# Mehooz/vision4leg

Measured on AMD Instinct MI355X. Metric: PPO env-steps/s (encoder+update, sim excluded), higher is better.
Workload: dtype f16; 1 GPU; ppo_locotransformer thin-goal: LocoTransformer S=93 A=6, E=32 envs x T=512, B=1024, 3 opt epochs; net=loco, envs_per_gpu=32, horizon=512, minibatch=1024, opt_epochs=3, parallelism=dp1, includes_rollout_inference=True, logp_old=recorded at action time (target_pf forward skipped; SURVEY 8d declared saving)

## Files before the change

vision4leg_amd/csrc/bwd.h:

```cpp
#pragma once
#include "infer.h"

namespace v4l {

struct BwdLayer {
  const void *w2t, *w1t, *wot, *wint;
  const float *g1, *g2;
  const float* dy;
  const float *s_qkv, *s_P, *s_xh1, *s_rs1, *s_xh2, *s_rs2;
  const void* s_f;
  void *o_dz2, *o_df, *o_dz1, *o_dqkv;
  float* o_dx;
  float *gp2, *bp2, *gp1, *bp1;
};

struct BwdLayerStack { BwdLayer l[2]; };

struct BwdHead {
  const void *w2t, *w1t, *w0t;
  const float* dout;
  const float *s_h1, *s_h0;
  float *o_dh1, *o_dh0;
};
struct BwdTail {
// ... 416 lines not shown
      f32x4 ap[2][2];
#pragma unroll
      for (int m = 0; m < 2; ++m)
#pragma unroll
        for (int nn = 0; nn < 2; ++nn) ap[m][nn] = f32x4{0.f, 0.f, 0.f, 0.f};
#pragma unroll
      for (int ks = 0; ks < 2; ++ks) {
        frag_t fa[2], fb[2];
#pragma unroll
        for (int m = 0; m < 2; ++m) {
          fa[m] = *reinterpret_cast<const frag_t*>(dC + (m * 16 + fr) * LY::LDA + ks * 32 + fg);
          fb[m] = *reinterpret_cast<const frag_t*>(Vv + (m * 16 + fr) * LY::LDA + ks * 32 + fg);
        }
#pragma unroll
        for (int m = 0; m < 2; ++m)
#pragma unroll
          for (int nn = 0; nn < 2; ++nn) mma_k32(ap[m][nn], fb[nn], fa[m]);
      }
#pragma unroll
      for (int m = 0; m < 2; ++m) {
        const int i = m * 16 + fr;
        float rd = 0.f;
#pragma unroll
        for (int nn = 0; nn < 2; ++nn)
#pragma unroll
          for (int r = 0; r < 4; ++r) {
            const bool ok = i < NTOK && nn * 16 + qr + r < NTOK;
            rd = fmaf(pp[m][nn][r], ok ? ap[m][nn][r] : 0.f, rd);
          }
        rd += __shfl_xor(rd, 16, 64);
        rd += __shfl_xor(rd, 32, 64);
#pragma unroll
        for (int nn = 0; nn < 2; ++nn) {
          float d[4];
#pragma unroll
          for (int r = 0; r < 4; ++r) {
            const bool ok = i < NTOK && nn * 16 + qr + r < NTOK;
            d[r] = ok ? pp[m][nn][r] * (ap[m][nn][r] - rd) : 0.f;
          }
          const int j0 = nn * 16 + qr;
          st4(dS + i * LY::LDK + j0, d[0], d[1], d[2], d[3]);
#pragma unroll
          for (int r = 0; r < 4; ++r) {
            dSt[(j0 + r) * LY::LDK + i] = (T)d[r];
            Pt[(j0 + r) * LY::LDK + i] = (T)pp[m][nn][r];
          }
        }
      }
      T* R = reinterpret_cast<T*>(aw);
      if (lane < LY::LDR * 2 / 16) *reinterpret_cast<uint4*>(R + NTOK * LY::LDR + lane * 8) = uint4{0u, 0u, 0u, 0u};
      T* og = reinterpret_cast<T*>(w.o_dqkv) + (row0 + wave * NTOK) * 192;
      auto product = [&](const T* A, const T* B, float scale, int coff) {
        f32x4 acc[2][4];
        frag_t fa[2], fb[4];
#pragma unroll
        for (int m = 0; m < 2; ++m) fa[m] = *reinterpret_cast<const frag_t*>(A + (m * 16 + fr) * LY::LDK + fg);
#pragma unroll
        for (int nn = 0; nn < 4; ++nn) fb[nn] = *reinterpret_cast<const frag_t*>(B + (nn * 16 + fr) * LY::LDK + fg);
#pragma unroll
        for (int m = 0; m < 2; ++m)
#pragma unroll
          for (int nn = 0; nn < 4; ++nn) {
            acc[m][nn] = f32x4{0.f, 0.f, 0.f, 0.f};
            mma_k32(acc[m][nn], fb[nn], fa[m]);
          }
#pragma unroll
        for (int m = 0; m < 2; ++m) {
          const int x = m * 16 + fr;
          if (x < NTOK) {
#pragma unroll
            for (int nn = 0; nn < 4; ++nn) {
              const float v0 = acc[m][nn][0] * scale, v1 = acc[m][nn][1] * scale, v2 = acc[m][nn][2] * scale, v3 = acc[m][nn][3] * scale;
              st4(R + x * LY::LDR + coff + nn * 16 + qr, v0, v1, v2, v3);
              st4(og + x * 192 + coff + nn * 16 + qr, v0, v1, v2, v3);
            }
          }
        }
      };
      product(dS, Kt, 0.125f, 0);
      product(dSt, Qt, 0.125f, TD);
      product(Pt, dCt, 1.f, 2 * TD);
    }
  } else {
    const bool act = wave < ns;
    float* qs = big + wave * NTOK * LY::LDQ;
    float* p = sp + wave * NTOK * ATT_PLD;
    float* ds = sp + (SPW + wave) * NTOK * ATT_PLD;
    const float* dc = a + wave * NTOK * LY::LDX;
    if (act) {
      if (lane < 54) {
        const int a2 = lane / 6, b3 = lane - a2 * 6;
        const int i0 = 2 * a2, i1 = min(i0 + 1, NTOK - 1), j0 = 3 * b3, j1 = min(j0 + 1, NTOK - 1), j2 = min(j0 + 2, NTOK - 1);
        const float *da = dc + i0 * LY::LDX, *db = dc + i1 * LY::LDX;
        const float *va = qs + j0 * LY::LDQ + 2 * TD, *vb = qs + j1 * LY::LDQ + 2 * TD, *vc = qs + j2 * LY::LDQ + 2 * TD;
        float s00 = 0.f, s01 = 0.f, s02 = 0.f, s10 = 0.f, s11 = 0.f, s12 = 0.f;
#pragma unroll 4
        for (int d = 0; d < TD; d += 4) {
          const float4 x0 = *reinterpret_cast<const float4*>(da + d), x1 = *reinterpret_cast<const float4*>(db + d);
          const float4 y0 = *reinterpret_cast<const float4*>(va + d), y1 = *reinterpret_cast<const float4*>(vb + d);
          const float4 y2 = *reinterpret_cast<const float4*>(vc + d);
          s00 = fmaf(x0.x, y0.x, s00); s00 = fmaf(x0.y, y0.y, s00); s00 = fmaf(x0.z, y0.z, s00); s00 = fmaf(x0.w, y0.w, s00);
          s01 = fmaf(x0.x, y1.x, s01); s01 = fmaf(x0.y, y1.y, s01); s01 = fmaf(x0.z, y1.z, s01); s01 = fmaf(x0.w, y1.w, s01);
          s02 = fmaf(x0.x, y2.x, s02); s02 = fmaf(x0.y, y2.y, s02); s02 = fmaf(x0.z, y2.z, s02); s02 = fmaf(x0.w, y2.w, s02);
          s10 = fmaf(x1.x, y0.x, s10); s10 = fmaf(x1.y, y0.y, s10); s10 = fmaf(x1.z, y0.z, s10); s10 = fmaf(x1.w, y0.w, s10);
          s11 = fmaf(x1.x, y1.x, s11); s11 = fmaf(x1.y, y1.y, s11); s11 = fmaf(x1.z, y1.z, s11); s11 = fmaf(x1.w, y1.w, s11);
          s12 = fmaf(x1.x, y2.x, s12); s12 = fmaf(x1.y, y2.y, s12); s12 = fmaf(x1.z, y2.z, s12); s12 = fmaf(x1.w, y2.w, s12);
        }
        float* r0 = ds + i0 * ATT_PLD;
        float* r1 = ds + i1 * ATT_PLD;
        r0[j0] = s00;
        if (j0 + 1 < NTOK) r0[j0 + 1] = s01;
        if (j0 + 2 < NTOK) r0[j0 + 2] = s02;
        if (i0 + 1 < NTOK) {
          r1[j0] = s10;
          if (j0 + 1 < NTOK) r1[j0 + 1] = s11;
          if (j0 + 2 < NTOK) r1[j0 + 2] = s12;
        }
      }
      if (lane < 3 * NTOK) {
        const int i = lane / 3, j = NTOK + lane - i * 3;
        p[i * ATT_PLD + j] = 0.f;
        ds[i * ATT_PLD + j] = 0.f;
      }
    }
    __syncthreads();
    if (act && lane < NTOK) {
      float rd = 0.f;
#pragma unroll
      for (int j = 0; j < NTOK; ++j) rd = fmaf(p[lane * ATT_PLD + j], ds[lane * ATT_PLD + j], rd);
#pragma unroll
      for (int j = 0; j < NTOK; ++j) {
        const float pj = p[lane * ATT_PLD + j];
        ds[lane * ATT_PLD + j] = rt<T>(pj * (ds[lane * ATT_PLD + j] - rd));
        p[lane * ATT_PLD + j] = rt<T>(pj);
      }
    }
    __syncthreads();
    if (act) {
      float dcr[NTOK], kr[NTOK], qq[NTOK], dq[NTOK], dk[NTOK], dv[NTOK];
#pragma unroll
      for (int i = 0; i < NTOK; ++i) {
        dcr[i] = dc[i * LY::LDX + lane];
        qq[i] = qs[i * LY::LDQ + lane];
        kr[i] = qs[i * LY::LDQ + TD + lane];
        dq[i] = dk[i] = dv[i] = 0.f;
      }
#pragma unroll
      for (int i = 0; i < NTOK; ++i) {
        float pi[ATT_PLD], si[ATT_PLD];
#pragma unroll
        for (int j4 = 0; j4 < ATT_PLD; j4 += 4) {
          const float4 pv = *reinterpret_cast<const float4*>(p + i * ATT_PLD + j4);
          const float4 sv = *reinterpret_cast<const float4*>(ds + i * ATT_PLD + j4);
          pi[j4] = pv.x; pi[j4 + 1] = pv.y; pi[j4 + 2] = pv.z; pi[j4 + 3] = pv.w;
          si[j4] = sv.x; si[j4 + 1] = sv.y; si[j4 + 2] = sv.z; si[j4 + 3] = sv.w;
        }
#pragma unroll
        for (int j = 0; j < NTOK; ++j) {
          dv[j] = fmaf(pi[j], dcr[i], dv[j]);
          dq[i] = fmaf(si[j], kr[j], dq[i]);
          dk[j] = fmaf(si[j], qq[i], dk[j]);
        }
      }
      T* og = reinterpret_cast<T*>(w.o_dqkv) + (row0 + wave * NTOK) * 192;
#pragma unroll
      for (int i = 0; i < NTOK; ++i) {
        const float q8 = dq[i] * 0.125f, k8 = dk[i] * 0.125f;
        qs[i * LY::LDQ + lane] = q8;
        qs[i * LY::LDQ + TD + lane] = k8;
        qs[i * LY::LDQ + 2 * TD + lane] = dv[i];
        og[i * 192 + lane] = (T)q8;
        og[i * 192 + TD + lane] = (T)k8;
        og[i * 192 + 2 * TD + lane] = (T)dv[i];
      }
    }
  }
  __syncthreads();
  LAY_STAMP(7);
  {
    f32x4 acc[MT][1];
    zero_acc(acc);
    if constexpr (LY::MFMA_ATT) {
      typedef typename Frag<T>::type frag_t;
      const int fg = (lane >> 4) * 8;
      const T* rp[MT];
#pragma unroll
      for (int mt = 0; mt < MT; ++mt) {
        const int row = mt * 16 + fr, sm = row / NTOK, t = row - sm * NTOK;
        rp[mt] = row < nrows ? reinterpret_cast<const T*>(att + (size_t)sm * LY::att_w) + t * LY::LDR
                             : reinterpret_cast<const T*>(att) + NTOK * LY::LDR;
      }
#pragma unroll
      for (int ks = 0; ks < 6; ++ks)
#pragma unroll
        for (int mt = 0; mt < MT; ++mt)
          mma_k32(acc[mt][0], ring_dxin.fb[ks][0], *reinterpret_cast<const frag_t*>(rp[mt] + ks * 32 + fg));
    } else {
      block_gemm<T, MT, 1, 6>(acc, big, LY::LDQ, (const T*)w.wint, 192, nt1, lane, ring_dxin);
    }
    const int n4 = wave * 16 + qr;
#pragma unroll
    for (int mt = 0; mt < MT; ++mt) {
      const int row = mt * 16 + fr;
      const float4 r = *reinterpret_cast<const float4*>(b + row * LY::LDX + n4);
      acc[mt][0][0] += r.x; acc[mt][0][1] += r.y; acc[mt][0][2] += r.z; acc[mt][0][3] += r.w;
      if (row < nrows) st4(w.o_dx + (row0 + row) * TD + n4, acc[mt][0][0], acc[mt][0][1], acc[mt][0][2], acc[mt][0][3]);
      if (TAIL && last) st4(at + row * LY::LDX + n4, acc[mt][0][0], acc[mt][0][1], acc[mt][0][2], acc[mt][0][3]);
    }
    if (!last) {
      if constexpr (LY::MFMA_ATT) __syncthreads();
#pragma unroll
      for (int mt = 0; mt < MT; ++mt)
        st4(a + (mt * 16 + fr) * LY::LDX + n4, acc[mt][0][0], acc[mt][0][1], acc[mt][0][2], acc[mt][0][3]);
    }
  }
  pre2 = pre2_next;
  LAY_STAMP(8);
  }
  if constexpr (TAIL) {
    __syncthreads();
    {
      f32x4 acc[MT][1];
      zero_acc(acc);
      block_gemm<T, MT, 1, 2>(acc, at, LY::LDX, (const T*)tl.wupt, 64, nt1, lane, ring_up);
      const int n4 = wave * 16 + qr;
#pragma unroll
      for (int mt = 0; mt < MT; ++mt) {
        const int row = mt * 16 + fr;
        const int sm = row / NTOK, t = row - sm * NTOK;
        const bool ok = row < nrows && t > 0;
        const int64_t o = ok ? ((int64_t)(s0 + sm) * 16 + (t - 1)) * TD + n4 : 0;
        const float4 m = tm_c3[mt];
        if (ok)
          st4(tl.o_dc3 + o, m.x > 0.f ? acc[mt][0][0] : 0.f, m.y > 0.f ? acc[mt][0][1] : 0.f, m.z > 0.f ? acc[mt][0][2] : 0.f,
              m.w > 0.f ? acc[mt][0][3] : 0.f);
      }
    }
    float* dt = big;
    T* dh = reinterpret_cast<T*>(big + 16 * LY::LDX);
    GemmRing<T, 4, 8> ring_f2 = gemm_prefetch<T, 4, 8>((const T*)tl.wf2t, 256, nt4, lane);
    __syncthreads();
#pragma unroll
    for (int k = 0; k < 4; ++k) {
      const int idx = tid + k * 256, r = idx >> 6, c = idx & 63;
      dt[r * LY::LDX + c] = r < ns && tm_x0[k] > 0.f ? at[(r * NTOK) * LY::LDX + c] : 0.f;
    }
    __syncthreads();
    f32x4 acc[1][4];
    auto masked = [&](const float4 (&m)[4], T* dst, float* save) {
      const bool ok = fr < ns;
#pragma unroll
      for (int j = 0; j < 4; ++j) {
        const int n4 = nt4[j] * 16 + qr;
        const float d0 = m[j].x > 0.f ? acc[0][j][0] : 0.f, d1 = m[j].y > 0.f ? acc[0][j][1] : 0.f;
        const float d2 = m[j].z > 0.f ? acc[0][j][2] : 0.f, d3 = m[j].w > 0.f ? acc[0][j][3] : 0.f;
        if (dst != nullptr) st4(dst + fr * LY::LDF + n4, d0, d1, d2, d3);
        if (ok) st4(save + (int64_t)(s0 + fr) * 256 + n4, d0, d1, d2, d3);
      }
    };
    zero_acc(acc);
    block_gemm<T, 1, 4, 2>(acc, dt, LY::LDX, (const T*)tl.wpt, 64, nt4, lane, ring_pr);
    masked(tm_e1, dh, tl.o_dhc);
    __syncthreads();
    zero_acc(acc);
    block_gemm<T, 1, 4, 8>(acc, dh, LY::LDF, (const T*)tl.wf2t, 256, nt4, lane, ring_f2);
    masked(tm_e0, (T*)nullptr, tl.o_de0);
  }
  LAY_STAMP(9);
}


struct BwdConv {
  const void* w3d;
  const void* w2d[4];
  const void* image;
  const int* rowidx;
  const float *c1, *c2;
  const float* dc3;
  float *slab1, *slab2, *slab3;
  float *bslab1, *bslab2, *bslab3;
  int n;
  void *t_dc2, *t_dc1;
};
template <typename T> struct BwdConvLds {
  static constexpr bool B16 = sizeof(T) == 2;
  static constexpr int LF = 64 + 4;
  static constexpr int LC1 = 32 + (B16 ? 8 : 0);
  static constexpr int IMGP = B16 ? 1 : 2;
  static constexpr int LT = 64 + (B16 ? 8 : 4);
  static constexpr int LP2 = 64 + (B16 ? 8 : 4);
  static constexpr int LP1 = 256 + (B16 ? 8 : 4);
  static constexpr size_t dc3_b = (size_t)17 * LT * sizeof(T);
  static constexpr size_t c2_b = (size_t)36 * LF * 4;
  static constexpr size_t dc2_b = (size_t)48 * LT * sizeof(T);
  static constexpr size_t dc2T_b = (size_t)64 * LP2 * sizeof(T);
  static constexpr size_t c1_b = ((size_t)225 * LC1 * sizeof(T) + 15) / 16 * 16;
  static constexpr size_t dc1_b = (size_t)32 * LP1 * sizeof(T);
  static constexpr size_t img_b = (size_t)(4 / IMGP) * 4096 * sizeof(T);
  static constexpr size_t w2_b = B16 ? (size_t)4 * 32 * 256 * sizeof(T) : 0;
  static constexpr size_t bytes = dc3_b + c2_b + dc2_b + dc2T_b + c1_b + dc1_b + img_b + w2_b;
  static_assert(bytes <= 160 * 1024, "one block per CU");
};

template <typename T> __device__ __forceinline__ typename Frag<T>::type frag_of(const float (&v)[8]) {
  typename Frag<T>::type f;
  if constexpr (sizeof(T) == 2) {
#pragma unroll
    for (int j = 0; j < 8; ++j) f[j] = (T)v[j];
  } else {
#pragma unroll
    for (int j = 0; j < 8; ++j) f.v[j] = v[j];
  }
  return f;
}
template <typename H>
__device__ __forceinline__ typename Frag<H>::type frag_of_t(const H (&v)[8]) {
  static_assert(sizeof(H) == 2, "16-bit operand type");
  typename Frag<H>::type f;
#pragma unroll
  for (int j = 0; j < 8; ++j) f[j] = v[j];
  return f;
}
__device__ __forceinline__ f32x8 frag_of_t(const float (&v)[8]) { return frag_of<float>(v); }

template <typename T, int MT, int NT, int KS, int KS0 = 0, int PDEPTH = 4, class RowF>
__device__ __forceinline__ void gather_gemm(f32x4 (&acc)[MT][NT], const T* __restrict__ W, int Kp, int nt0, int lane, RowF arow) {
  typedef typename Frag<T>::type frag_t;
  constexpr int PD = NT >= 2 ? 2 : (KS < PDEPTH ? KS : PDEPTH);
  const int fr = lane & 15, fg = (lane >> 4) * 8;
  const T* wrow = W + (int64_t)(nt0 * 16 + fr) * Kp + fg + KS0 * 32;
  frag_t fb[PD][NT];
#pragma unroll
  for (int d = 0; d < PD; ++d)
#pragma unroll
    for (int j = 0; j < NT; ++j) fb[d][j] = *reinterpret_cast<const frag_t*>(wrow + (int64_t)j * 16 * Kp + d * 32);
#pragma unroll
  for (int ks = 0; ks < KS; ++ks) {
    frag_t cur[NT];
#pragma unroll
    for (int j = 0; j < NT; ++j) cur[j] = fb[ks % PD][j];
    if (ks + PD < KS) {
#pragma unroll
      for (int j = 0; j < NT; ++j) fb[ks % PD][j] = *reinterpret_cast<const frag_t*>(wrow + (int64_t)j * 16 * Kp + (ks + PD) * 32);
    }
#pragma unroll
    for (int mt = 0; mt < MT; ++mt) {
      const frag_t fa = *reinterpret_cast<const frag_t*>(arow(mt, (ks + KS0) >> 1) + ((ks + KS0) & 1) * 32 + fg);
#pragma unroll
      for (int j = 0; j < NT; ++j)
        mma_k32(acc[mt][j], cur[j], fa);
    }
  }
}

#ifdef V4L_INFER_TIMING
#define CONV_STAMP(i) do { if (blockIdx.x == 0 && threadIdx.x == 0 && smp == 3 * (int)gridDim.x) g_inf_stamps[16 + (i)] = clock64(); } while (0)
#else
#define CONV_STAMP(i)
#endif
template <typename T, bool A16 = false>
__global__ __launch_bounds__(512) void bwd_conv_kernel(BwdConv a) {
  static_assert(!A16 || sizeof(T) == 2, "A16: activations saved in the bf16 operand type");
  typedef BwdConvLds<T> LY;
  typedef typename Frag<T>::type frag_t;
  constexpr int NTH = 512;
  extern __shared__ __attribute__((aligned(16))) unsigned char smem[];
  T* sdc3 = reinterpret_cast<T*>(smem);
  float* sc2 = reinterpret_cast<float*>(smem + LY::dc3_b);
  T* sdc2t = reinterpret_cast<T*>(smem + LY::dc3_b + LY::c2_b);
  T* sdc2T = reinterpret_cast<T*>(smem + LY::dc3_b + LY::c2_b + LY::dc2_b);
  constexpr size_t o_c1 = LY::dc3_b + LY::c2_b + LY::dc2_b + LY::dc2T_b;
  T* sc1 = reinterpret_cast<T*>(smem + o_c1);
  T* sdc1T = reinterpret_cast<T*>(smem + o_c1 + LY::c1_b);
  T* simg = reinterpret_cast<T*>(smem + o_c1 + LY::c1_b + LY::dc1_b);
  T* sw2 = reinterpret_cast<T*>(smem + o_c1 + LY::c1_b + LY::dc1_b + LY::img_b);
  const int tid = threadIdx.x, lane = tid & 63, wave = tid >> 6;
  const int fr = lane & 15, g = lane >> 4, qr = g * 4;
  const int kt2 = wave * 4;
  const int ch1 = wave >> 1, th1 = wave & 1;
  f32x4 acc2[4][4], acc1[2][2];
#pragma unroll
  for (int t = 0; t < 4; ++t) {
#pragma unroll
    for (int c = 0; c < 4; ++c) acc2[t][c] = f32x4{0.f, 0.f, 0.f, 0.f};
    acc1[t >> 1][t & 1] = f32x4{0.f, 0.f, 0.f, 0.f};
  }
  float b2r[4] = {0.f, 0.f, 0.f, 0.f};
  float b1r[4] = {0.f, 0.f, 0.f, 0.f};
  for (int i = tid; i < 12 * LY::LT; i += NTH) sdc2t[36 * LY::LT + i] = (T)0.f;
  for (int i = tid; i < 64 * LY::LP2; i += NTH) sdc2T[i] = (T)0.f;
  for (int i = tid; i < 32 * LY::LP1; i += NTH) sdc1T[i] = (T)0.f;
  for (int i = tid; i < LY::LT; i += NTH) sdc3[16 * LY::LT + i] = (T)0.f;
  constexpr int CH = 4 / LY::IMGP;

  constexpr int V = 16 / sizeof(T);
  constexpr int N4 = 225 * 8, PT = (N4 + NTH - 1) / NTH;
  constexpr int N8 = 225 * 4, PT8 = (N8 + NTH - 1) / NTH;
  typedef typename Frag<T>::type chunk_t;
  float4 hv0 = float4{0.f, 0.f, 0.f, 0.f}, hv1 = hv0, cv[A16 ? 1 : PT];
  chunk_t h16 = {}, c16[A16 ? PT8 : 1] = {};
  auto load_next = [&](int sm) {
    const float* g3 = a.dc3 + (int64_t)sm * 16 * 64;
    if constexpr (A16) {
      const chunk_t* g2 = reinterpret_cast<const chunk_t*>(reinterpret_cast<const T*>(a.c2) + (int64_t)sm * 36 * 64);
      const chunk_t* g1 = reinterpret_cast<const chunk_t*>(reinterpret_cast<const T*>(a.c1) + (int64_t)sm * 225 * 32);
      h16 = g2[tid < 288 ? tid : 0];
      if (tid >= 256) hv1 = *reinterpret_cast<const float4*>(g3 + (tid - 256) * 4);
#pragma unroll
      for (int k = 0; k < PT8; ++k) {
        const int i8 = tid + k * NTH;
        c16[k] = g1[i8 < N8 ? i8 : 0];
      }
    } else {
      const float* g2 = a.c2 + (int64_t)sm * 36 * 64;
      const float* g1 = a.c1 + (int64_t)sm * 225 * 32;
      hv0 = *reinterpret_cast<const float4*>(g2 + tid * 4);
      if (tid >= 256) hv1 = *reinterpret_cast<const float4*>(g3 + (tid - 256) * 4);
      else if (tid < 64) hv1 = *reinterpret_cast<const float4*>(g2 + (512 + tid) * 4);
#pragma unroll
      for (int k = 0; k < PT; ++k) {
        const int i4 = tid + k * NTH;
        cv[k] = *reinterpret_cast<const float4*>(g1 + (i4 < N4 ? i4 : 0) * 4);
      }
    }
  };
  auto store_next = [&]() {
    if constexpr (A16) {
      if (tid < 288) {
        float* d = sc2 + (tid >> 3) * LY::LF + (tid & 7) * 8;
        *reinterpret_cast<float4*>(d) = float4{(float)h16[0], (float)h16[1], (float)h16[2], (float)h16[3]};
        *reinterpret_cast<float4*>(d + 4) = float4{(float)h16[4], (float)h16[5], (float)h16[6], (float)h16[7]};
      }
      if (tid >= 256) st4(sdc3 + ((tid - 256) >> 4) * LY::LT + (tid & 15) * 4, hv1.x, hv1.y, hv1.z, hv1.w);
#pragma unroll
      for (int k = 0; k < PT8; ++k) {
        const int i8 = tid + k * NTH;
        if (i8 < N8) *reinterpret_cast<chunk_t*>(sc1 + (i8 >> 2) * LY::LC1 + (i8 & 3) * 8) = c16[k];
      }
    } else {
      *reinterpret_cast<float4*>(sc2 + (tid >> 4) * LY::LF + (tid & 15) * 4) = hv0;
      if (tid >= 256) st4(sdc3 + ((tid - 256) >> 4) * LY::LT + (tid & 15) * 4, hv1.x, hv1.y, hv1.z, hv1.w);
      else if (tid < 64) *reinterpret_cast<float4*>(sc2 + (32 + (tid >> 4)) * LY::LF + (tid & 15) * 4) = hv1;
#pragma unroll
      for (int k = 0; k < PT; ++k) {
        const int i4 = tid + k * NTH;
        if (i4 < N4) st4(sc1 + (i4 >> 3) * LY::LC1 + (i4 & 7) * 4, cv[k].x, cv[k].y, cv[k].z, cv[k].w);
      }
    }
  };
  {
    const bool first = (int)blockIdx.x < a.n;
    if (first) load_next(blockIdx.x);
    if constexpr (LY::B16) {
      float4 wv[4096 / NTH];
#pragma unroll
      for (int k = 0; k < 4096 / NTH; ++k) {
        const int c = tid + k * NTH, k8 = c & 31, n = (c >> 5) & 31, cl = c >> 10;
        wv[k] = *reinterpret_cast<const float4*>(reinterpret_cast<const T*>(a.w2d[cl]) + n * 256 + k8 * 8);
      }
#pragma unroll
      for (int k = 0; k < 4096 / NTH; ++k) {
        const int c = tid + k * NTH, k8 = c & 31, n = (c >> 5) & 31, cl = c >> 10;
        const int dst = ((cl * 2 + (n >> 4)) * 8 + (k8 >> 2)) * 64 + (k8 & 3) * 16 + (n & 15);
        *reinterpret_cast<float4*>(sw2 + dst * 8) = wv[k];
      }
    }
    if (first) store_next();
  }
  for (int smp = blockIdx.x; smp < a.n; smp += gridDim.x) {
    __syncthreads();
    CONV_STAMP(0);
    const int64_t slot = a.rowidx != nullptr ? a.rowidx[smp] : smp;
    const T* gimg = reinterpret_cast<const T*>(a.image) + slot * 16384;
    CONV_STAMP(1);
    {
      const int nt = wave & 3;
      const T* W = reinterpret_cast<const T*>(a.w3d);
      int iy[3], ix[3];
      bool okr[3];
#pragma unroll
      for (int m = 0; m < 3; ++m) {
        const int px = m * 16 + fr;
        okr[m] = px < 36;
        iy[m] = px / 6; ix[m] = px - iy[m] * 6;
      }
      f32x4 acc[3][1];
#pragma unroll
      for (int m = 0; m < 3; ++m) acc[m][0] = f32x4{0.f, 0.f, 0.f, 0.f};
      auto arow = [&](int m, int tap) -> const T* {
        const int ta = tap / 3, tb = tap - ta * 3;
        const int oy = iy[m] - ta, ox = ix[m] - tb;
        const bool ok = okr[m] && oy >= 0 && oy < 4 && ox >= 0 && ox < 4;
        return sdc3 + (ok ? oy * 4 + ox : 16) * LY::LT;
      };
      float4* part = reinterpret_cast<float4*>(simg);
      if (wave >= 4) {
        gather_gemm<T, 3, 1, 9, 9, LY::B16 ? 9 : 3>(acc, W, 576, nt, lane, arow);
#pragma unroll
        for (int m = 0; m < 3; ++m) part[(nt * 3 + m) * 64 + lane] = float4{acc[m][0][0], acc[m][0][1], acc[m][0][2], acc[m][0][3]};
      } else {
        gather_gemm<T, 3, 1, 9, 0, LY::B16 ? 9 : 3>(acc, W, 576, nt, lane, arow);
      }
      __syncthreads();
      if (wave < 4) {
#pragma unroll
        for (int m = 0; m < 3; ++m) {
          const int px = m * 16 + fr, c4 = nt * 16 + qr;
          if (px < 36) {
            const float4 hi = part[(nt * 3 + m) * 64 + lane];
            const float4 mk = *reinterpret_cast<const float4*>(sc2 + px * LY::LF + c4);
            const float d0 = mk.x > 0.f ? acc[m][0][0] + hi.x : 0.f, d1 = mk.y > 0.f ? acc[m][0][1] + hi.y : 0.f;
            const float d2 = mk.z > 0.f ? acc[m][0][2] + hi.z : 0.f, d3 = mk.w > 0.f ? acc[m][0][3] + hi.w : 0.f;
            st4(sdc2t + px * LY::LT + c4, d0, d1, d2, d3);
            if (a.t_dc2 != nullptr) st4(reinterpret_cast<T*>(a.t_dc2) + ((int64_t)smp * 36 + px) * 64 + c4, d0, d1, d2, d3);
            T* tp = sdc2T + c4 * LY::LP2 + px;
            tp[0] = (T)d0; tp[LY::LP2] = (T)d1; tp[2 * LY::LP2] = (T)d2; tp[3 * LY::LP2] = (T)d3;
            b2r[0] += d0; b2r[1] += d1; b2r[2] += d2; b2r[3] += d3;
          }
        }
      }
    }
    __syncthreads();
    CONV_STAMP(2);
#pragma unroll
    for (int k = 0; k < CH * 4096 / V / NTH; ++k)
      __builtin_amdgcn_global_load_lds((const V4L_GLOBAL void*)(gimg + (int64_t)(tid + k * NTH) * V),
                                       (__attribute__((address_space(3))) void*)(simg + ((tid & ~63) + k * NTH) * V), 16, 0, 0);
#pragma unroll
    for (int st = 0; st < 2; ++st) {
      frag_t fy[4];
#pragma unroll
      for (int c = 0; c < 4; ++c) fy[c] = *reinterpret_cast<const frag_t*>(sdc2T + (c * 16 + fr) * LY::LP2 + st * 32 + g * 8);
#pragma unroll
      for (int t = 0; t < 4; ++t) {
        const int kt = kt2 + t, tap = kt >> 1, ci = (kt & 1) * 16 + fr;
        const int ky = tap >> 2, kx = tap & 3;
        T w[8];
#pragma unroll
        for (int j = 0; j < 8; ++j) {
          const int pos = st * 32 + g * 8 + j;
          const int pp = pos < 36 ? pos : 0, oy = pp / 6, ox = pp - oy * 6;
          w[j] = sc1[((2 * oy + ky) * 15 + 2 * ox + kx) * LY::LC1 + ci];
        }
        const frag_t fx = frag_of_t(w);
#pragma unroll
        for (int c = 0; c < 4; ++c) mma_k32(acc2[t][c], fx, fy[c]);
      }
    }
    CONV_STAMP(3);
    {
      const int cls = wave >> 1, py = cls >> 1, pxx = cls & 1, nh = wave & 1;
      const int nIy = (15 - py + 1) >> 1, nIx = (15 - pxx + 1) >> 1;
      int ry[4], rx[4];
#pragma unroll
      for (int m = 0; m < 4; ++m) { const int r = m * 16 + fr; ry[m] = r >> 3; rx[m] = r & 7; }
      f32x4 acc[4][1];
#pragma unroll
      for (int m = 0; m < 4; ++m) acc[m][0] = f32x4{0.f, 0.f, 0.f, 0.f};
      auto arow = [&](int m, int tap) -> const T* {
        const int oy = ry[m] - (tap >> 1), ox = rx[m] - (tap & 1);
        const bool ok = ry[m] < nIy && rx[m] < nIx && oy >= 0 && oy < 6 && ox >= 0 && ox < 6;
        return sdc2t + (ok ? oy * 6 + ox : 36) * LY::LT;
      };
      if constexpr (LY::B16) {
        const T* wl = sw2 + (cls * 2 + nh) * 8 * 512 + lane * 8;
#pragma unroll
        for (int ks = 0; ks < 8; ++ks) {
          const frag_t fw = *reinterpret_cast<const frag_t*>(wl + ks * 512);
#pragma unroll
          for (int m = 0; m < 4; ++m)
            mma_k32(acc[m][0], fw, *reinterpret_cast<const frag_t*>(arow(m, ks >> 1) + (ks & 1) * 32 + g * 8));
        }
      } else {
        gather_gemm<T, 4, 1, 8>(acc, reinterpret_cast<const T*>(a.w2d[cls]), 256, nh, lane, arow);
      }
#pragma unroll
      for (int m = 0; m < 4; ++m) {
        if (ry[m] < nIy && rx[m] < nIx) {
          const int p = (py + 2 * ry[m]) * 15 + pxx + 2 * rx[m];
          const int c4 = nh * 16 + qr;
          const float4 mk = ld4(sc1 + p * LY::LC1 + c4);
          const float d0 = mk.x > 0.f ? acc[m][0][0] : 0.f, d1 = mk.y > 0.f ? acc[m][0][1] : 0.f;
          const float d2 = mk.z > 0.f ? acc[m][0][2] : 0.f, d3 = mk.w > 0.f ? acc[m][0][3] : 0.f;
          T* tp = sdc1T + c4 * LY::LP1 + p;
          tp[0] = (T)d0; tp[LY::LP1] = (T)d1; tp[2 * LY::LP1] = (T)d2; tp[3 * LY::LP1] = (T)d3;
          if (a.t_dc1 != nullptr) st4(reinterpret_cast<T*>(a.t_dc1) + ((int64_t)smp * 225 + p) * 32 + c4, d0, d1, d2, d3);
          b1r[0] += d0; b1r[1] += d1; b1r[2] += d2; b1r[3] += d3;
        }
      }
    }
    __syncthreads();
    CONV_STAMP(4);
    CONV_STAMP(5);
    const bool more = smp + (int)gridDim.x < a.n;
    if (more) load_next(smp + gridDim.x);
#pragma unroll 1
    for (int h = 0; h < LY::IMGP; ++h) {
      if (h > 0) {
        __syncthreads();
        for (int i = tid; i < CH * 4096 / V; i += NTH)
          *reinterpret_cast<float4*>(simg + i * V) = *reinterpret_cast<const float4*>(gimg + (int64_t)h * CH * 4096 + i * V);
        __syncthreads();
      }
      if (ch1 >= h * CH && ch1 < (h + 1) * CH) {
        const T* ich = simg + (ch1 - h * CH) * 4096;
#pragma unroll 1
        for (int st = 0; st < 8; ++st) {
          frag_t fy[2];
#pragma unroll
          for (int c = 0; c < 2; ++c) fy[c] = *reinterpret_cast<const frag_t*>(sdc1T + (c * 16 + fr) * LY::LP1 + st * 32 + g * 8);
          int po2[8];
#pragma unroll
          for (int j = 0; j < 8; ++j) {
            const int pos = st * 32 + g * 8 + j;
            const int pp = pos < 225 ? pos : 0, oy = pp / 15, ox = pp - oy * 15;
            po2[j] = (4 * oy) * 64 + 4 * ox;
          }
#pragma unroll
          for (int tt = 0; tt < 2; ++tt) {
            const int ky = (th1 * 2 + tt) * 2 + (fr >> 3), kx = fr & 7;
            T w[8];
#pragma unroll
            for (int j = 0; j < 8; ++j) w[j] = ich[po2[j] + ky * 64 + kx];
            const frag_t fx = frag_of_t(w);
#pragma unroll
            for (int c = 0; c < 2; ++c) mma_k32(acc1[c][tt], fx, fy[c]);
          }
        }
      }
    }
    if (more) store_next();
    CONV_STAMP(6);
  }
  {
    float* o2 = a.slab2 + (int64_t)blockIdx.x * 64 * 512;
#pragma unroll
    for (int t = 0; t < 4; ++t)
#pragma unroll
      for (int c = 0; c < 4; ++c)
        *reinterpret_cast<float4*>(o2 + (c * 16 + fr) * 512 + (kt2 + t) * 16 + qr) =
            float4{acc2[t][c][0], acc2[t][c][1], acc2[t][c][2], acc2[t][c][3]};
    float* o1 = a.slab1 + (int64_t)blockIdx.x * 32 * 256;
#pragma unroll
    for (int c = 0; c < 2; ++c)
#pragma unroll
      for (int tt = 0; tt < 2; ++tt)
        *reinterpret_cast<float4*>(o1 + (c * 16 + fr) * 256 + (ch1 * 4 + th1 * 2 + tt) * 16 + qr) =
            float4{acc1[c][tt][0], acc1[c][tt][1], acc1[c][tt][2], acc1[c][tt][3]};
    __syncthreads();
    float* red2 = reinterpret_cast<float*>(sdc1T);
    float* red1 = red2 + 64 * 16;
    static_assert(LY::dc1_b >= (64 * 16 + 32 * 64) * 4, "bias reduction scratch");
    if (wave < 4) {
#pragma unroll
      for (int i = 0; i < 4; ++i) red2[((wave & 3) * 16 + qr + i) * 16 + fr] = b2r[i];
    }
#pragma unroll
    for (int i = 0; i < 4; ++i) red1[((wave & 1) * 16 + qr + i) * 64 + (wave >> 1) * 16 + fr] = b1r[i];
    __syncthreads();
    if (tid < 64) {
      float t = 0.f;
#pragma unroll
      for (int k = 0; k < 16; ++k) t += red2[tid * 16 + k];
      a.bslab2[(int64_t)blockIdx.x * 64 + tid] = t;
    }
    if (tid < 32) {
      float t = 0.f;
#pragma unroll 8
      for (int k = 0; k < 64; ++k) t += red1[tid * 64 + k];
      a.bslab1[(int64_t)blockIdx.x * 32 + tid] = t;
    }
  }
}

template <typename T, bool A16 = false>
__global__ __launch_bounds__(256) void bwd_conv3_wgrad_kernel(BwdConv a) {
  typedef typename Frag<T>::type frag_t;
  constexpr int LF = 64 + 4;
  __shared__ __attribute__((aligned(16))) float sdc3[16 * LF];
  __shared__ __attribute__((aligned(16))) float sc2[36 * LF];
  const int tid = threadIdx.x, lane = tid & 63, wave = tid >> 6;
  const int fr = lane & 15, g = lane >> 4, qr = g * 4;
  const int kt3 = wave * 9;
  f32x4 acc3[9][4];
#pragma unroll
  for (int t = 0; t < 9; ++t)
#pragma unroll
    for (int c = 0; c < 4; ++c) acc3[t][c] = f32x4{0.f, 0.f, 0.f, 0.f};
  float bias3 = 0.f;
  int x_base[9], x_pos[8];
#pragma unroll
  for (int t = 0; t < 9; ++t) {
    const int kt = kt3 + t, tap = kt >> 2, ky = tap / 3, kx = tap - ky * 3;
    x_base[t] = (ky * 6 + kx) * LF + (kt & 3) * 16 + fr;
  }
#pragma unroll
  for (int j = 0; j < 8; ++j) {
    const int pos = (g & 1) * 8 + j;
    x_pos[j] = ((pos >> 2) * 6 + (pos & 3)) * LF;
  }
  const int i2 = tid + 512 < 36 * 16 ? tid + 512 : 0;
  float4 r3 = {0.f, 0.f, 0.f, 0.f}, r2a = r3, r2b = r3, r2c = r3;
  typedef typename Frag<T>::type chunk_t;
  chunk_t q2a = {}, q2b = {};
  auto fetch = [&](int sm) {
    const float* g3 = a.dc3 + (int64_t)sm * 16 * 64;
    r3 = *reinterpret_cast<const float4*>(g3 + tid * 4);
    if constexpr (A16) {
      const chunk_t* g2 = reinterpret_cast<const chunk_t*>(reinterpret_cast<const T*>(a.c2) + (int64_t)sm * 36 * 64);
      q2a = g2[tid];
      q2b = g2[tid < 32 ? 256 + tid : 0];
    } else {
      const float* g2 = a.c2 + (int64_t)sm * 36 * 64;
      r2a = *reinterpret_cast<const float4*>(g2 + tid * 4);
      r2b = *reinterpret_cast<const float4*>(g2 + (tid + 256) * 4);
      r2c = *reinterpret_cast<const float4*>(g2 + i2 * 4);
    }
  };
  auto file = [&]() {
    *reinterpret_cast<float4*>(sdc3 + (tid >> 4) * LF + (tid & 15) * 4) = r3;
    if constexpr (A16) {
      auto put = [&](int j, const chunk_t& q) {
        float* d = sc2 + (j >> 3) * LF + (j & 7) * 8;
        *reinterpret_cast<float4*>(d) = float4{(float)q[0], (float)q[1], (float)q[2], (float)q[3]};
        *reinterpret_cast<float4*>(d + 4) = float4{(float)q[4], (float)q[5], (float)q[6], (float)q[7]};
      };
      put(tid, q2a);
      if (tid < 32) put(256 + tid, q2b);
    } else {
      *reinterpret_cast<float4*>(sc2 + (tid >> 4) * LF + (tid & 15) * 4) = r2a;
      *reinterpret_cast<float4*>(sc2 + ((tid + 256) >> 4) * LF + (tid & 15) * 4) = r2b;
      if (tid + 512 < 36 * 16) *reinterpret_cast<float4*>(sc2 + ((tid + 512) >> 4) * LF + (tid & 15) * 4) = r2c;
    }
  };
  if ((int)blockIdx.x < a.n) fetch(blockIdx.x);
  for (int smp = blockIdx.x; smp < a.n; smp += gridDim.x) {
    __syncthreads();
    file();
    const int nxt = smp + (int)gridDim.x;
    if (nxt < a.n) fetch(nxt);
    __syncthreads();
    if (tid < 64) {
      float t = 0.f;
#pragma unroll
      for (int p = 0; p < 16; ++p) t += sdc3[p * LF + tid];
      bias3 += t;
    }
    float v[8];
    frag_t fy[4];
#pragma unroll
    for (int c = 0; c < 4; ++c) {
#pragma unroll
      for (int j = 0; j < 8; ++j) {
        const float x = sdc3[((g & 1) * 8 + j) * LF + c * 16 + fr];
        v[j] = g < 2 ? x : 0.f;
      }
      fy[c] = frag_of<T>(v);
    }
#pragma unroll
    for (int t = 0; t < 9; ++t) {
#pragma unroll
      for (int j = 0; j < 8; ++j) {
        const float x = sc2[x_base[t] + x_pos[j]];
        v[j] = g < 2 ? x : 0.f;
      }
      const frag_t fx = frag_of<T>(v);
#pragma unroll
      for (int c = 0; c < 4; ++c) mma_k32(acc3[t][c], fx, fy[c]);
    }
  }
  float* o3 = a.slab3 + (int64_t)blockIdx.x * 64 * 576;
#pragma unroll
  for (int t = 0; t < 9; ++t)
#pragma unroll
    for (int c = 0; c < 4; ++c)
      *reinterpret_cast<float4*>(o3 + (c * 16 + fr) * 576 + (kt3 + t) * 16 + qr) =
          float4{acc3[t][c][0], acc3[t][c][1], acc3[t][c][2], acc3[t][c][3]};
  if (tid < 64) a.bslab3[(int64_t)blockIdx.x * 64 + tid] = bias3;
}

}
```

Before: 410,000 env-steps/s.

## Repack conv1 input image in LDS for vectorized im2col weight-gradient fragments

```diff
diff --git a/vision4leg_amd/csrc/bwd.h b/vision4leg_amd/csrc/bwd.h
--- a/vision4leg_amd/csrc/bwd.h
+++ b/vision4leg_amd/csrc/bwd.h
@@ -742,6 +742,8 @@
   static_assert(bytes <= 160 * 1024, "one block per CU");
 };
 
+typedef __attribute__((ext_vector_type(4))) uint32_t u32x4;
+
 template <typename T> __device__ __forceinline__ typename Frag<T>::type frag_of(const float (&v)[8]) {
   typename Frag<T>::type f;
   if constexpr (sizeof(T) == 2) {
@@ -840,50 +842,54 @@
   float4 hv0 = float4{0.f, 0.f, 0.f, 0.f}, hv1 = hv0, cv[A16 ? 1 : PT];
   chunk_t h16 = {}, c16[A16 ? PT8 : 1] = {};
   auto load_next = [&](int sm) {
-    const float* g3 = a.dc3 + (int64_t)sm * 16 * 64;
+    uint32_t t = tid;
+    asm volatile("" : "+v"(t));
+    const char* g3 = reinterpret_cast<const char*>(a.dc3 + (int64_t)sm * 16 * 64);
     if constexpr (A16) {
-      const chunk_t* g2 = reinterpret_cast<const chunk_t*>(reinterpret_cast<const T*>(a.c2) + (int64_t)sm * 36 * 64);
-      const chunk_t* g1 = reinterpret_cast<const chunk_t*>(reinterpret_cast<const T*>(a.c1) + (int64_t)sm * 225 * 32);
-      h16 = g2[tid < 288 ? tid : 0];
-      if (tid >= 256) hv1 = *reinterpret_cast<const float4*>(g3 + (tid - 256) * 4);
+      const char* g2 = reinterpret_cast<const char*>(reinterpret_cast<const T*>(a.c2) + (int64_t)sm * 36 * 64);
+      const char* g1 = reinterpret_cast<const char*>(reinterpret_cast<const T*>(a.c1) + (int64_t)sm * 225 * 32);
+      h16 = *reinterpret_cast<const chunk_t*>(g2 + (t < 288u ? t : 0u) * 16u);
+      if (tid >= 256) hv1 = *reinterpret_cast<const float4*>(g3 + (t - 256u) * 16u);
 #pragma unroll
       for (int k = 0; k < PT8; ++k) {
-        const int i8 = tid + k * NTH;
-        c16[k] = g1[i8 < N8 ? i8 : 0];
+        const uint32_t i8 = t + k * NTH;
+        c16[k] = *reinterpret_cast<const chunk_t*>(g1 + (i8 < (uint32_t)N8 ? i8 : 0u) * 16u);
       }
     } else {
-      const float* g2 = a.c2 + (int64_t)sm * 36 * 64;
-      const float* g1 = a.c1 + (int64_t)sm * 225 * 32;
-      hv0 = *reinterpret_cast<const float4*>(g2 + tid * 4);
-      if (tid >= 256) hv1 = *reinterpret_cast<const float4*>(g3 + (tid - 256) * 4);
-      else if (tid < 64) hv1 = *reinterpret_cast<const float4*>(g2 + (512 + tid) * 4);
+      const char* g2 = reinterpret_cast<const char*>(a.c2 + (int64_t)sm * 36 * 64);
+      const char* g1 = reinterpret_cast<const char*>(a.c1 + (int64_t)sm * 225 * 32);
+      hv0 = *reinterpret_cast<const float4*>(g2 + t * 16u);
+      if (tid >= 256) hv1 = *reinterpret_cast<const float4*>(g3 + (t - 256u) * 16u);
+      else if (tid < 64) hv1 = *reinterpret_cast<const float4*>(g2 + (512u + t) * 16u);
 #pragma unroll
       for (int k = 0; k < PT; ++k) {
-        const int i4 = tid + k * NTH;
-        cv[k] = *reinterpret_cast<const float4*>(g1 + (i4 < N4 ? i4 : 0) * 4);
+        const uint32_t i4 = t + k * NTH;
+        cv[k] = *reinterpret_cast<const float4*>(g1 + (i4 < (uint32_t)N4 ? i4 : 0u) * 16u);
       }
     }
   };
   auto store_next = [&]() {
+    int t = tid;
+    asm volatile("" : "+v"(t));
     if constexpr (A16) {
-      if (tid < 288) {
-        float* d = sc2 + (tid >> 3) * LY::LF + (tid & 7) * 8;
+      if (t < 288) {
+        float* d = sc2 + (t >> 3) * LY::LF + (t & 7) * 8;
         *reinterpret_cast<float4*>(d) = float4{(float)h16[0], (float)h16[1], (float)h16[2], (float)h16[3]};
         *reinterpret_cast<float4*>(d + 4) = float4{(float)h16[4], (float)h16[5], (float)h16[6], (float)h16[7]};
       }
-      if (tid >= 256) st4(sdc3 + ((tid - 256) >> 4) * LY::LT + (tid & 15) * 4, hv1.x, hv1.y, hv1.z, hv1.w);
+      if (t >= 256) st4(sdc3 + ((t - 256) >> 4) * LY::LT + (t & 15) * 4, hv1.x, hv1.y, hv1.z, hv1.w);
 #pragma unroll
       for (int k = 0; k < PT8; ++k) {
-        const int i8 = tid + k * NTH;
+        const int i8 = t + k * NTH;
         if (i8 < N8) *reinterpret_cast<chunk_t*>(sc1 + (i8 >> 2) * LY::LC1 + (i8 & 3) * 8) = c16[k];
       }
     } else {
-      *reinterpret_cast<float4*>(sc2 + (tid >> 4) * LY::LF + (tid & 15) * 4) = hv0;
-      if (tid >= 256) st4(sdc3 + ((tid - 256) >> 4) * LY::LT + (tid & 15) * 4, hv1.x, hv1.y, hv1.z, hv1.w);
-      else if (tid < 64) *reinterpret_cast<float4*>(sc2 + (32 + (tid >> 4)) * LY::LF + (tid & 15) * 4) = hv1;
+      *reinterpret_cast<float4*>(sc2 + (t >> 4) * LY::LF + (t & 15) * 4) = hv0;
+      if (t >= 256) st4(sdc3 + ((t - 256) >> 4) * LY::LT + (t & 15) * 4, hv1.x, hv1.y, hv1.z, hv1.w);
+      else if (t < 64) *reinterpret_cast<float4*>(sc2 + (32 + (t >> 4)) * LY::LF + (t & 15) * 4) = hv1;
 #pragma unroll
       for (int k = 0; k < PT; ++k) {
-        const int i4 = tid + k * NTH;
+        const int i4 = t + k * NTH;
         if (i4 < N4) st4(sc1 + (i4 >> 3) * LY::LC1 + (i4 & 7) * 4, cv[k].x, cv[k].y, cv[k].z, cv[k].w);
       }
     }
@@ -952,7 +958,12 @@
             const float d0 = mk.x > 0.f ? acc[m][0][0] + hi.x : 0.f, d1 = mk.y > 0.f ? acc[m][0][1] + hi.y : 0.f;
             const float d2 = mk.z > 0.f ? acc[m][0][2] + hi.z : 0.f, d3 = mk.w > 0.f ? acc[m][0][3] + hi.w : 0.f;
             st4(sdc2t + px * LY::LT + c4, d0, d1, d2, d3);
-            if (a.t_dc2 != nullptr) st4(reinterpret_cast<T*>(a.t_dc2) + ((int64_t)smp * 36 + px) * 64 + c4, d0, d1, d2, d3);
+            if (a.t_dc2 != nullptr) {
+              uint32_t t = tid;
+              asm volatile("" : "+v"(t));
+              const uint32_t o = (m * 16 + (t & 15)) * 64 + ((t >> 6) & 3) * 16 + ((t >> 4) & 3) * 4;
+              st4(reinterpret_cast<T*>(a.t_dc2) + (int64_t)smp * 36 * 64 + o, d0, d1, d2, d3);
+            }
             T* tp = sdc2T + c4 * LY::LP2 + px;
             tp[0] = (T)d0; tp[LY::LP2] = (T)d1; tp[2 * LY::LP2] = (T)d2; tp[3 * LY::LP2] = (T)d3;
             b2r[0] += d0; b2r[1] += d1; b2r[2] += d2; b2r[3] += d3;
@@ -1022,11 +1033,35 @@
           const float4 mk = ld4(sc1 + p * LY::LC1 + c4);
           const float d0 = mk.x > 0.f ? acc[m][0][0] : 0.f, d1 = mk.y > 0.f ? acc[m][0][1] : 0.f;
           const float d2 = mk.z > 0.f ? acc[m][0][2] : 0.f, d3 = mk.w > 0.f ? acc[m][0][3] : 0.f;
-          T* tp = sdc1T + c4 * LY::LP1 + p;
+          T* tp = sdc1T + c4 * LY::LP1 + (LY::B16 ? (py + 2 * ry[m]) * 16 + pxx + 2 * rx[m] : p);
           tp[0] = (T)d0; tp[LY::LP1] = (T)d1; tp[2 * LY::LP1] = (T)d2; tp[3 * LY::LP1] = (T)d3;
-          if (a.t_dc1 != nullptr) st4(reinterpret_cast<T*>(a.t_dc1) + ((int64_t)smp * 225 + p) * 32 + c4, d0, d1, d2, d3);
+          if (a.t_dc1 != nullptr) {
+            uint32_t t = tid;
+            asm volatile("" : "+v"(t));
+            const uint32_t r = m * 16 + (t & 15), pp = (((t >> 8) & 1) + 2 * (r >> 3)) * 15 + ((t >> 7) & 1) + 2 * (r & 7);
+            const uint32_t o = pp * 32 + ((t >> 6) & 1) * 16 + ((t >> 4) & 3) * 4;
+            st4(reinterpret_cast<T*>(a.t_dc1) + (int64_t)smp * 225 * 32 + o, d0, d1, d2, d3);
+          }
           b1r[0] += d0; b1r[1] += d1; b1r[2] += d2; b1r[3] += d3;
         }
+      }
+    }
+    if constexpr (LY::B16) {
+      asm volatile("s_waitcnt vmcnt(0)" ::: "memory");
+      T* hrow = simg + (wave * 64 + (lane >> 4) * NTH) * V + (lane & 15) * 32;
+      u32x4 q[4];
+#pragma unroll
+      for (int i = 0; i < 4; ++i) q[i] = reinterpret_cast<const u32x4*>(hrow)[i];
+      T* drow = simg + (wave * 64 + (lane >> 4) * NTH) * V + ((lane & 15) >> 1) * 64 + (lane & 1) * 8;
+#pragma unroll
+      for (int b = 0; b < 4; ++b) {
+        u32x4 o;
+#pragma unroll
+        for (int k = 0; k < 4; ++k) {
+          const uint32_t lo = q[k][b >> 1], hi = q[k][2 + (b >> 1)];
+          o[k] = (b & 1) ? (lo >> 16) | (hi & 0xffff0000u) : (lo & 0xffffu) | (hi << 16);
+        }
+        *reinterpret_cast<u32x4*>(drow + b * 16) = o;
       }
     }
     __syncthreads();
@@ -1034,6 +1069,28 @@
     CONV_STAMP(5);
     const bool more = smp + (int)gridDim.x < a.n;
     if (more) load_next(smp + gridDim.x);
+    if constexpr (LY::B16) {
+      const T* ich = simg + ch1 * 4096 + (th1 * 4 + (fr >> 3)) * 64 + (fr & 3) * 16 + (g & 1) * 8;
+      const int sh = ((fr >> 2) & 1) * 16, ro = (g >> 1) * 256;
+#pragma unroll 1
+      for (int st = 0; st < 8; ++st) {
+        frag_t fy[2];
+#pragma unroll
+        for (int c = 0; c < 2; ++c) fy[c] = *reinterpret_cast<const frag_t*>(sdc1T + (c * 16 + fr) * LY::LP1 + st * 32 + g * 8);
+        const T* src = ich + st * 512 + (st < 7 ? ro : 0);
+#pragma unroll
+        for (int tt = 0; tt < 2; ++tt) {
+          const u32x4 d = *reinterpret_cast<const u32x4*>(src + tt * 128);
+          const uint32_t e = *reinterpret_cast<const uint32_t*>(src + tt * 128 + 8);
+          u32x4 f;
+          f[0] = __builtin_amdgcn_alignbit(d[1], d[0], sh); f[1] = __builtin_amdgcn_alignbit(d[2], d[1], sh);
+          f[2] = __builtin_amdgcn_alignbit(d[3], d[2], sh); f[3] = __builtin_amdgcn_alignbit(e, d[3], sh);
+          const frag_t fx = __builtin_bit_cast(frag_t, f);
+#pragma unroll
+          for (int c = 0; c < 2; ++c) mma_k32(acc1[c][tt], fx, fy[c]);
+        }
+      }
+    } else {
 #pragma unroll 1
     for (int h = 0; h < LY::IMGP; ++h) {
       if (h > 0) {
@@ -1068,6 +1125,7 @@
           }
         }
       }
+    }
     }
     if (more) store_next();
     CONV_STAMP(6);
```

New measurement: 393,600 env-steps/s. -4.0%, worse.
